# arneschneuing/DiffSBDD

Hardware: NVIDIA H100
Metric: ligand_atoms_per_sec_500step_ddpm (higher is better)
Workload: dtype f32

## Files before the change

### diffsbdd_b200/csrc/dsb_tc.cu

```cuda
#include "dsb_tc.cuh"

namespace dsb {
using namespace tc;

__global__ void pack_b_image_kernel(float* __restrict__ hi, float* __restrict__ lo, const float* __restrict__ src, int lds,
                                    int scol, int n_rows, int n_dst_off, int K, int chunks, int TN) {
  const int64_t idx = (int64_t)blockIdx.x * blockDim.x + threadIdx.x;
  if (idx >= (int64_t)n_rows * K) return;
  const int n = (int)(idx / K), k = (int)(idx - (int64_t)n * K);
  const int nd = n_dst_off + n, nt = nd / TN, nl = nd % TN;
  const int kc = k / TKC, c = (k % TKC) >> 2, j = k & 3;
  const size_t off = ((size_t)nt * chunks + kc) * (size_t)(TN * TKC) + sw128_offset(nl, c) / 4 + j;
  const float w = src[(size_t)n * lds + scol + k];
  const float h = tf32_hi(w);
  hi[off] = h;
  lo[off] = w - h;
}

void launch_pack_b_image(float* hi, float* lo, const float* src, int lds, int scol, int n_rows, int n_dst_off, int K, int tn) {
  const int64_t tot = (int64_t)n_rows * K;
  pack_b_image_kernel<<<(unsigned)((tot + 255) / 256), 256>>>(hi, lo, src, lds, scol, n_rows, n_dst_off, K, K / TKC, tn);
}

__global__ void pack_b_image_f16_kernel(__half* __restrict__ hi, __half* __restrict__ lo, const float* __restrict__ src, int lds,
                                        int scol, int n_rows, int n_dst_off, int K, int chunks, float scale, int TN) {
  const int64_t idx = (int64_t)blockIdx.x * blockDim.x + threadIdx.x;
  if (idx >= (int64_t)n_rows * K) return;
  const int n = (int)(idx / K), k = (int)(idx - (int64_t)n * K);
  const int nd = n_dst_off + n, nt = nd / TN, nl = nd % TN;
  const int kc = k / TKC16, c16 = (k % TKC16) >> 3, j = k & 7;
  const size_t off = ((size_t)nt * chunks + kc) * (size_t)(TN * 64) + sw128_offset(nl, c16) / 2 + j;
  const float w = src[(size_t)n * lds + scol + k] * scale;
  const __half h = __float2half_rn(w);
  hi[off] = h;
  lo[off] = __float2half_rn(w - __half2float(h));
}

void launch_pack_b_image_f16(float* hi, float* lo, const float* src, int lds, int scol, int n_rows, int n_dst_off, int K, float scale, int tn) {
  const int64_t tot = (int64_t)n_rows * K;
  pack_b_image_f16_kernel<<<(unsigned)((tot + 255) / 256), 256>>>(reinterpret_cast<__half*>(hi), reinterpret_cast<__half*>(lo), src,
                                                                  lds, scol, n_rows, n_dst_off, K, K / TKC16, scale, tn);
}

__global__ void absmax_kernel(const float* __restrict__ src, int lds, int scol, int n_rows, int K, unsigned* __restrict__ out) {
  const int64_t idx = (int64_t)blockIdx.x * blockDim.x + threadIdx.x;
  float v = 0.f;
  if (idx < (int64_t)n_rows * K) { const int n = (int)(idx / K), k = (int)(idx - (int64_t)n * K); v = fabsf(src[(size_t)n * lds + scol + k]); }
#pragma unroll
  for (int o = 16; o > 0; o >>= 1) v = fmaxf(v, __shfl_xor_sync(0xffffffffu, v, o));
  if ((threadIdx.x & 31) == 0) atomicMax(out, __float_as_uint(v));
}
void launch_absmax(const float* src, int lds, int scol, int n_rows, int K, unsigned* out) {
  const int64_t tot = (int64_t)n_rows * K;
  absmax_kernel<<<(unsigned)((tot + 255) / 256), 256>>>(src, lds, scol, n_rows, K, out);
}

constexpr size_t kControlBytes = 128;
static_assert(sizeof(Control) <= kControlBytes, "Control block grew");
__device__ __forceinline__ char* align1024(uint8_t* raw) {
  return reinterpret_cast<char*>(raw) + ((1024u - (smem_u32(raw) & 1023u)) & 1023u);
}
template <int H> constexpr size_t tc_smem_base() { return 1024 + (size_t)NSTAGE * Geo<H>::STAGE_BYTES + kControlBytes; }

struct TcGemmArgs {
  const float* A1; int lda1; int K1;
  const float* A2; int lda2; int K2; float div2; const int32_t* deg2;
  const float* Bhi; const float* Blo;
  const float* bias; const float* R; int ldr;
  float* C; int ldc; int M; int Nn; int act;
  float* Z; int ldz;
  int dead_mt; int dead_nt;
  float inv_scale;
};

struct TileMap {
  int ntn, ntm, dead_mt, dead_nt, nA, n_live;
  __device__ TileMap(int M, int Nn, int dmt, int dnt, int TN) {
    ntn = Nn / TN; ntm = (M + TM - 1) / TM;
    dead_nt = dnt; dead_mt = dnt > 0 ? (dmt < ntm ? dmt : ntm) : ntm;
    nA = dead_mt * ntn;
    n_live = nA + (ntm - dead_mt) * (ntn - dead_nt);
  }
  __device__ void get(int t, int& mt, int& nt) const {
    if (t < nA) { mt = t / ntn; nt = t - mt * ntn; }
    else { const int u = t - nA, w = ntn - dead_nt; mt = dead_mt + u / w; nt = dead_nt + (u - (u / w) * w); }
  }
};

template <TcFormat FMT, int H>
__global__ void __launch_bounds__(TC_THREADS, 1) tc_node_gemm_kernel(TcGemmArgs g) {
  using G = Geo<H>;
  constexpr bool F16 = FMT != TcFormat::TF32x3;
  constexpr int TN = H, HPC = F16 ? 2 : 1;
  extern __shared__ uint8_t smem_raw[];
  char* const stages = align1024(smem_raw);
  Control* ctl = reinterpret_cast<Control*>(stages + NSTAGE * G::STAGE_BYTES);
  const int wg = threadIdx.x >> 7, warp = (threadIdx.x >> 5) & 3, lane = threadIdx.x & 31;
  const TileMap tm(g.M, g.Nn, g.dead_mt, g.dead_nt, TN);
  const int n_tiles = tm.n_live;
  const int n_my = ((int)blockIdx.x < n_tiles) ? (n_tiles - (int)blockIdx.x + (int)gridDim.x - 1) / (int)gridDim.x : 0;
  if (n_my == 0) return;
  const int K = g.K1 + g.K2, chunks = K / (F16 ? TKC16 : TKC);
  const uint32_t total = (uint32_t)(n_my * chunks);
  pdl_trigger();
  if (threadIdx.x == 0) control_init(ctl);
  __syncthreads();
  pdl_wait();
  const WeightStream<FMT, H> wst{ctl, stages};
  auto issue_w = [&](uint32_t q) {
    const int it = (int)(q / chunks), kc = (int)(q - (uint32_t)it * chunks);
    int mt, nt;
    tm.get(blockIdx.x + it * gridDim.x, mt, nt);
    const size_t off = ((size_t)nt * chunks + kc) * G::B_CHUNK_FLOATS;
    wst.issue(q, g.Bhi + off, g.Blo + off);
  };
  if (threadIdx.x >= MMA_THREADS) {
    regs_dec<WEIGHT_WG_REGS>();
    if (threadIdx.x == MMA_THREADS)
      for (uint32_t q = 0; q < total; ++q) issue_w(q);
    return;
  }
  regs_inc<MMA_WG_REGS>();

  const int sr = lane >> 3, pc = lane & 7;
  const int r0 = wg * WG_ROWS + 16 * warp + 4 * sr;
  const int re = wg * WG_ROWS + 16 * warp + (lane >> 2);
  const bool divides = g.div2 != 1.0f || g.deg2 != nullptr;
  float acc[G::ACC];
  MmaTracker trk;
  uint32_t q = 0;
  for (int it = 0; it < n_my; ++it) {
    int mt, nt;
    tm.get(blockIdx.x + it * gridDim.x, mt, nt);
    const int m0 = mt * TM, n0 = nt * TN;
    for (int kc = 0; kc < chunks; ++kc, ++q) {
      const int s = q & 1;
      char* st = stages + (size_t)s * G::STAGE_BYTES;
#pragma unroll
      for (int h = 0; h < HPC; ++h) {
        const int hf = kc * HPC + h, k = hf * TKC + 4 * pc;
        const bool second = k >= g.K1;
        float4 v[4];
#pragma unroll
        for (int i = 0; i < 4; ++i) {
          const int m = m0 + r0 + i;
          v[i] = make_float4(0.f, 0.f, 0.f, 0.f);
          if (m < g.M) v[i] = second ? *reinterpret_cast<const float4*>(g.A2 + (size_t)m * g.lda2 + (k - g.K1))
                                     : *reinterpret_cast<const float4*>(g.A1 + (size_t)m * g.lda1 + k);
        }
#pragma unroll
        for (int i = 0; i < 4; ++i) {
          float4 x = v[i];
          if (second && divides) {
            const int m = m0 + r0 + i;
            const float dv = g.deg2 ? (float)max(m < g.M ? g.deg2[m] : 1, 1) : g.div2;
            x.x = __fdiv_rn(x.x, dv); x.y = __fdiv_rn(x.y, dv); x.z = __fdiv_rn(x.z, dv); x.w = __fdiv_rn(x.w, dv);
          }
          store_pair<FMT>(st + piece_offset<F16>(r0 + i, hf, pc), pk2(x.x, x.y), pk2(x.z, x.w));
        }
      }
      fence_proxy_async();
      wg_sync(wg);
      mbar_wait(&ctl->full_w[s], (q >> 1) & 1);
      wgmma_fence();
      mma_chunk<FMT, H>(acc, st, wg, kc == 0);
      wgmma_commit();
      trk.release_prev(ctl, (int)q, lane == 0);
    }
    trk.drain<H>(ctl, acc, lane == 0);
    const f32x2 ip = pk2(g.inv_scale, g.inv_scale);
#pragma unroll
    for (int j = 0; j < H / 8; ++j) {
      const int n = n0 + 8 * j + 2 * (lane & 3);
      const f32x2 b = g.bias ? *reinterpret_cast<const float2*>(g.bias + n) : pk2(0.f, 0.f);
#pragma unroll
      for (int hh = 0; hh < 2; ++hh) {
        f32x2 x = pk2(acc[4 * j + 2 * hh], acc[4 * j + 2 * hh + 1]);
        x = F16 ? fma2(x, ip, b) : add2(x, b);
        if (g.act == 1) x = silu2(x);
        upk2(x, acc[4 * j + 2 * hh], acc[4 * j + 2 * hh + 1]);
      }
    }
    if (g.R) {
#pragma unroll
      for (int j = 0; j < H / 8; ++j) {
        const int n = n0 + 8 * j + 2 * (lane & 3);
#pragma unroll
        for (int hh = 0; hh < 2; ++hh) {
          const int row = min(m0 + re + 8 * hh, g.M - 1);
          const f32x2 x = add2(*reinterpret_cast<const float2*>(g.R + (size_t)row * g.ldr + n),
                               pk2(acc[4 * j + 2 * hh], acc[4 * j + 2 * hh + 1]));
          upk2(x, acc[4 * j + 2 * hh], acc[4 * j + 2 * hh + 1]);
        }
      }
    }
    acc_fence(acc);
#pragma unroll
    for (int j = 0; j < H / 8; ++j) {
      const int n = n0 + 8 * j + 2 * (lane & 3);
#pragma unroll
      for (int hh = 0; hh < 2; ++hh) {
        const int row = m0 + re + 8 * hh;
        if (row < g.M) {
          *reinterpret_cast<float2*>(g.C + (size_t)row * g.ldc + n) = pk2(acc[4 * j + 2 * hh], acc[4 * j + 2 * hh + 1]);
          if (g.Z) *reinterpret_cast<float2*>(g.Z + (size_t)row * g.ldz + n) = make_float2(0.f, 0.f);
        }
      }
    }
  }
}

struct EdgeScalars {
  float d2[TM], d0[TM];
  int row[TM], col[TM], type[TM];
  float dir[3][TM];
};

template <int H>
struct EdgeExtra {
  float vec[2][3 * H];
  float wa[H];
  EdgeScalars sc[2];
};

struct TcEdgeArgs {
  const float* P; int ldp;
  const float4* x; const float4* cent; const int32_t* gid;
  const int32_t* vrow_ptr; const int32_t* vmap; int n_rows;
  const int32_t *erow, *ecol; const float* ed0; int NL;
  int nm;
  const float* W2hi[2]; const float* W2lo[2];
  const float* wr[2]; const float* wr0[2]; const float* tb[2]; const float* b2[2];
  const float* wa; const float* ba;
  float norm_constant, coords_range; int use_tanh;
  float* agg;
  float4* xagg;
  float inv_scale[2];
  float* part;
  int vcap;
};

template <bool COORD>
struct ScalarSteps {
  int e, r, c, gi;
  float d0;
  float4 xi, xj;
  __device__ __forceinline__ void step(int k, const TcEdgeArgs& a, EdgeScalars* sc, int pr, int v0, int V, int m) {
    if (k == 0) {
      const int vr = v0 + pr;
      e = a.vmap[min(vr, V - 1)];
      e = vr < V ? e : -1;
    } else if (k == 1) {
      const int ec = max(e, 0);
      r = a.erow[ec]; c = a.ecol[ec]; d0 = a.ed0[ec];
      r = e >= 0 ? r : 0; c = e >= 0 ? c : 0;
    } else if (k == 2) {
      xi = a.x[r]; xj = a.x[c];
      if (COORD) gi = a.gid[r];
    } else {
      const bool live = e >= 0;
      const float dx = xi.x - xj.x, dy = xi.y - xj.y, dz = xi.z - xj.z;
      const float d2 = dx * dx + dy * dy + dz * dz;
      const int ty = (r < a.NL) == (c < a.NL) ? (r < a.NL ? 1 : 2) : 0;
      sc->row[pr] = live ? r : -1; sc->col[pr] = c; sc->d2[pr] = live ? d2 : 0.f; sc->d0[pr] = live ? d0 : 0.f;
      sc->type[pr] = live ? ty : 0;
      if (COORD) {
        float dir[3];
        if (m == 0) {
          const float den = sqrtf(d2 + 1e-8f) + a.norm_constant;
          dir[0] = dx / den; dir[1] = dy / den; dir[2] = dz / den;
        } else {
          const float4 mu = a.cent[gi];
          const float ax = xi.x - mu.x, ay = xi.y - mu.y, az = xi.z - mu.z;
          const float bx = xj.x - mu.x, by = xj.y - mu.y, bz = xj.z - mu.z;
          const float cx = ay * bz - az * by, cy = az * bx - ax * bz, cz = ax * by - ay * bx;
          const float cn = sqrtf(cx * cx + cy * cy + cz * cz) + a.norm_constant;
          dir[0] = cx / cn; dir[1] = cy / cn; dir[2] = cz / cn;
        }
#pragma unroll
        for (int k = 0; k < 3; ++k) sc->dir[k][pr] = live ? dir[k] : 0.f;
      }
    }
  }
};

template <bool COORD, TcFormat FMT, int H, bool TB, bool DET = false>
__global__ void __launch_bounds__(TC_THREADS, 1) tc_edge_kernel(TcEdgeArgs a) {
  using G = Geo<H>;
  constexpr bool F16 = FMT != TcFormat::TF32x3;
  constexpr int HPC = F16 ? 2 : 1;
  constexpr int chunks = H / (TKC * HPC);
  extern __shared__ uint8_t smem_raw[];
  char* const stages = align1024(smem_raw);
  Control* ctl = reinterpret_cast<Control*>(stages + NSTAGE * G::STAGE_BYTES);
  EdgeExtra<H>* ex = reinterpret_cast<EdgeExtra<H>*>(reinterpret_cast<char*>(ctl) + kControlBytes);
  const int wg = threadIdx.x >> 7, wt = threadIdx.x & 127, warp = (threadIdx.x >> 5) & 3, lane = threadIdx.x & 31;
  const int nm = a.nm;

  pdl_trigger();
  for (int i = threadIdx.x; i < H; i += TC_THREADS) {
    for (int m = 0; m < nm; ++m) {
      float* v = ex->vec[m];
      v[i] = a.wr[m][i]; v[H + i] = a.wr0[m][i]; v[2 * H + i] = a.b2[m][i];
    }
    ex->wa[i] = a.wa ? a.wa[i] : 0.f;
  }
  if (threadIdx.x == 0) control_init(ctl);
  __syncthreads();
  pdl_wait();
  const int E = DET ? min(a.vrow_ptr[a.n_rows], a.vcap) : a.vrow_ptr[a.n_rows];
  const int n_units = ((E + TM - 1) / TM) * nm;
  const int n_my = ((int)blockIdx.x < n_units) ? (n_units - (int)blockIdx.x + (int)gridDim.x - 1) / (int)gridDim.x : 0;
  if (n_my == 0) return;
  auto unit_tile = [&](int j, int& m) { const int v = blockIdx.x + j * gridDim.x, t = v / nm; m = v - t * nm; return t; };
  const uint32_t total = (uint32_t)(n_my * chunks);
  const WeightStream<FMT, H> wst{ctl, stages};
  auto issue_w = [&](uint32_t q) {
    const int j = (int)(q / chunks), kc = (int)(q - (uint32_t)j * chunks);
    int m;
    unit_tile(j, m);
    wst.issue(q, a.W2hi[m] + (size_t)kc * G::B_CHUNK_FLOATS, a.W2lo[m] + (size_t)kc * G::B_CHUNK_FLOATS);
  };
  if (threadIdx.x >= MMA_THREADS) {
    regs_dec<WEIGHT_WG_REGS>();
    if (threadIdx.x == MMA_THREADS)
      for (uint32_t q = 0; q < total; ++q) issue_w(q);
    return;
  }
  regs_inc<MMA_WG_REGS>();

  const bool has_att = (!COORD) && a.wa != nullptr;
  const float ba = has_att ? a.ba[0] : 0.f;
  const int sr = lane >> 3, pc = lane & 7;
  const int r0 = wg * WG_ROWS + 16 * warp + 4 * sr;
  const int re = wg * WG_ROWS + 16 * warp + (lane >> 2);
  const float* const Pt = a.P + 4 * pc;
  const int soff = nm * H;
  auto build = [&](const EdgeScalars* sc, int m, int kc, int s) {
    char* st = stages + (size_t)s * G::STAGE_BYTES;
    const int moff = m * H;
    const float* pr = Pt + (size_t)max(sc->row[r0], 0) * a.ldp + moff;
    const int4 cl = *reinterpret_cast<const int4*>(sc->col + r0);
    const float4 d2v = *reinterpret_cast<const float4*>(sc->d2 + r0), d0v = *reinterpret_cast<const float4*>(sc->d0 + r0);
    const int4 tyv = *reinterpret_cast<const int4*>(sc->type + r0);
    const float* const ps[4] = {Pt + (size_t)cl.x * a.ldp + (soff + moff), Pt + (size_t)cl.y * a.ldp + (soff + moff),
                                Pt + (size_t)cl.z * a.ldp + (soff + moff), Pt + (size_t)cl.w * a.ldp + (soff + moff)};
    const float pd2[4] = {d2v.x, d2v.y, d2v.z, d2v.w}, pd0[4] = {d0v.x, d0v.y, d0v.z, d0v.w};
    const int pty[4] = {TB ? tyv.x * H : 0, TB ? tyv.y * H : 0, TB ? tyv.z * H : 0, TB ? tyv.w * H : 0};
    const float* wr = ex->vec[m] + 4 * pc;
    const float* wr0 = wr + H;
    const float* tbm = TB ? a.tb[m] + 4 * pc : nullptr;
#pragma unroll
    for (int h = 0; h < HPC; ++h) {
      const int hf = kc * HPC + h;
      const float4 ga = *reinterpret_cast<const float4*>(pr + hf * TKC);
      float4 gb[4];
#pragma unroll
      for (int i = 0; i < 4; ++i) gb[i] = *reinterpret_cast<const float4*>(ps[i] + hf * TKC);
      const float4 r4 = *reinterpret_cast<const float4*>(wr + hf * TKC);
      const float4 r04 = *reinterpret_cast<const float4*>(wr0 + hf * TKC);
      const f32x2 a01 = pk2(ga.x, ga.y), a23 = pk2(ga.z, ga.w);
#pragma unroll
      for (int i = 0; i < 4; ++i) {
        const f32x2 d2p = pk2(pd2[i], pd2[i]), d0p = pk2(pd0[i], pd0[i]);
        f32x2 u01 = fma2(d0p, pk2(r04.x, r04.y), fma2(d2p, pk2(r4.x, r4.y), add2(a01, pk2(gb[i].x, gb[i].y))));
        f32x2 u23 = fma2(d0p, pk2(r04.z, r04.w), fma2(d2p, pk2(r4.z, r4.w), add2(a23, pk2(gb[i].z, gb[i].w))));
        if (TB) {
          const float4 t4 = *reinterpret_cast<const float4*>(tbm + pty[i] + hf * TKC);
          u01 = add2(u01, pk2(t4.x, t4.y)); u23 = add2(u23, pk2(t4.z, t4.w));
        }
        silu_pair<(DSB_SILU_PAIR & 1) != 0, (DSB_SILU_QUAD & 1) != 0>(u01, u23);
        store_pair<FMT>(st + piece_offset<F16>(r0 + i, hf, pc), u01, u23);
      }
    }
  };
  float acc[G::ACC];
  MmaTracker trk;
  uint32_t q = 0;
  auto issue = [&](int kc) {
    const int s = q & 1;
    fence_proxy_async();
    wg_sync(wg);
    mbar_wait(&ctl->full_w[s], (q >> 1) & 1);
    wgmma_fence();
    mma_chunk<FMT, H>(acc, stages + (size_t)s * G::STAGE_BYTES, wg, kc == 0);
    wgmma_commit();
    trk.release_prev(ctl, (int)q, lane == 0);
    ++q;
  };
  static_assert(chunks >= 2, "the scalar steps of the next unit need at least one chunk before the last");
  constexpr int kSteps = 4;
  const int psc = wg * WG_ROWS + (wt & (WG_ROWS - 1));
  ScalarSteps<COORD> stp;
  int m;
  int e0 = unit_tile(0, m) * TM;
  for (int k = 0; k < kSteps; ++k) stp.step(k, a, &ex->sc[0], psc, e0, E, m);
  wg_sync(wg);
  build(&ex->sc[0], m, 0, 0);
  for (int j = 0; j < n_my; ++j) {
    const EdgeScalars* sc = &ex->sc[j & 1];
    EdgeScalars* sc_next = &ex->sc[(j + 1) & 1];
    int m_next;
    const int e0_next = unit_tile(j + 1, m_next) * TM;
#pragma unroll ((F16 && !(FMT == TcFormat::F16x1 && !COORD && TB && H == 256)) ? chunks : 1)
    for (int kc = 0; kc < chunks - 1; ++kc) {
      issue(kc);
      for (int k = kc * kSteps / (chunks - 1); k < (kc + 1) * kSteps / (chunks - 1); ++k)
        stp.step(k, a, sc_next, psc, e0_next, E, m_next);
      build(sc, m, kc + 1, q & 1);
    }
    issue(chunks - 1);
    build(sc_next, m_next, 0, q & 1);
    trk.drain<H>(ctl, acc, lane == 0);

    const float* b2 = ex->vec[m] + 2 * H;
    const f32x2 ip = pk2(a.inv_scale[m], a.inv_scale[m]);
    float s_lo = 0.f, s_hi = 0.f;
    if constexpr (DET) {
      static_assert((H / 8) % 2 == 0, "DET epilogue pairs column groups");
#pragma unroll
      for (int jj = 0; jj < H / 8; jj += 2) {
        const int c = 8 * jj + 2 * (lane & 3);
        const f32x2 b0 = *reinterpret_cast<const float2*>(b2 + c), b1 = *reinterpret_cast<const float2*>(b2 + c + 8);
        const float2 w0 = *reinterpret_cast<const float2*>(ex->wa + c), w1 = *reinterpret_cast<const float2*>(ex->wa + c + 8);
        f32x2 lo0 = pk2(acc[4 * jj], acc[4 * jj + 1]), lo1 = pk2(acc[4 * jj + 4], acc[4 * jj + 5]);
        f32x2 hi0 = pk2(acc[4 * jj + 2], acc[4 * jj + 3]), hi1 = pk2(acc[4 * jj + 6], acc[4 * jj + 7]);
        lo0 = F16 ? fma2(lo0, ip, b0) : add2(lo0, b0); lo1 = F16 ? fma2(lo1, ip, b1) : add2(lo1, b1);
        hi0 = F16 ? fma2(hi0, ip, b0) : add2(hi0, b0); hi1 = F16 ? fma2(hi1, ip, b1) : add2(hi1, b1);
        silu_pair<(DSB_SILU_PAIR & 2) != 0, (DSB_SILU_QUAD & 2) != 0>(lo0, lo1);
        silu_pair<(DSB_SILU_PAIR & 2) != 0, (DSB_SILU_QUAD & 2) != 0>(hi0, hi1);
        upk2(lo0, acc[4 * jj], acc[4 * jj + 1]); upk2(lo1, acc[4 * jj + 4], acc[4 * jj + 5]);
        upk2(hi0, acc[4 * jj + 2], acc[4 * jj + 3]); upk2(hi1, acc[4 * jj + 6], acc[4 * jj + 7]);
        s_lo = fmaf(lo0.y, w0.y, fmaf(lo0.x, w0.x, s_lo));
        s_lo = fmaf(lo1.y, w1.y, fmaf(lo1.x, w1.x, s_lo));
        s_hi = fmaf(hi0.y, w0.y, fmaf(hi0.x, w0.x, s_hi));
        s_hi = fmaf(hi1.y, w1.y, fmaf(hi1.x, w1.x, s_hi));
      }
    } else {
#pragma unroll
    for (int jj = 0; jj < H / 8; ++jj) {
      const int c = 8 * jj + 2 * (lane & 3);
      const f32x2 bb = *reinterpret_cast<const float2*>(b2 + c);
      const float2 ww = *reinterpret_cast<const float2*>(ex->wa + c);
      f32x2 lo = pk2(acc[4 * jj], acc[4 * jj + 1]), hi = pk2(acc[4 * jj + 2], acc[4 * jj + 3]);
      lo = F16 ? fma2(lo, ip, bb) : add2(lo, bb);
      hi = F16 ? fma2(hi, ip, bb) : add2(hi, bb);
      silu_pair<(DSB_SILU_PAIR & 2) != 0, (DSB_SILU_QUAD & 2) != 0>(lo, hi);
      upk2(lo, acc[4 * jj], acc[4 * jj + 1]); upk2(hi, acc[4 * jj + 2], acc[4 * jj + 3]);
      s_lo = fmaf(lo.y, ww.y, fmaf(lo.x, ww.x, s_lo));
      s_hi = fmaf(hi.y, ww.y, fmaf(hi.x, ww.x, s_hi));
    }
    }
    s_lo += __shfl_xor_sync(0xffffffffu, s_lo, 1); s_lo += __shfl_xor_sync(0xffffffffu, s_lo, 2);
    s_hi += __shfl_xor_sync(0xffffffffu, s_hi, 1); s_hi += __shfl_xor_sync(0xffffffffu, s_hi, 2);
    const int row_lo = sc->row[re], row_hi = sc->row[re + 8];
    const int crow_lo = sc->row[re & ~3], crow_hi = sc->row[(re + 8) & ~3];
    const bool chunk_lane = (lane & 12) == 0;
    if constexpr (!COORD) {
      float g_lo = has_att ? sigmoid_f(s_lo + ba) : 1.0f, g_hi = has_att ? sigmoid_f(s_hi + ba) : 1.0f;
      g_lo = row_lo >= 0 ? g_lo : 0.f;
      g_hi = row_hi >= 0 ? g_hi : 0.f;
      const bool hi_half = (lane & 4) != 0, odd_group = (lane & 8) != 0;
      const int crow = hi_half ? crow_hi : crow_lo;
      const int chunk_row = hi_half ? (re + 8) & ~3 : re & ~3;
      float* const dst = (DET ? a.part + (size_t)((e0 + chunk_row) / kRowChunk) * H : a.agg + (size_t)max(crow, 0) * H)
                         + 2 * (lane & 3) + (odd_group ? 8 : 0);
#pragma unroll
      for (int jj = 0; jj < H / 8; jj += 2) {
        const float lo[4] = {g_lo * acc[4 * jj], g_lo * acc[4 * jj + 1], g_lo * acc[4 * jj + 4], g_lo * acc[4 * jj + 5]};
        const float hi[4] = {g_hi * acc[4 * jj + 2], g_hi * acc[4 * jj + 3], g_hi * acc[4 * jj + 6], g_hi * acc[4 * jj + 7]};
        float t[4];
#pragma unroll
        for (int k = 0; k < 4; ++k) t[k] = (hi_half ? hi[k] : lo[k]) + __shfl_xor_sync(0xffffffffu, hi_half ? lo[k] : hi[k], 4);
        float u[2];
#pragma unroll
        for (int k = 0; k < 2; ++k) u[k] = (odd_group ? t[2 + k] : t[k]) + __shfl_xor_sync(0xffffffffu, odd_group ? t[k] : t[2 + k], 8);
        if constexpr (DET)
          asm volatile("st.global.v2.f32 [%0], {%1, %2};" ::"l"(dst + 8 * jj), "f"(u[0]), "f"(u[1]) : "memory");
        else
          asm volatile("red.global.add.v2.f32 [%0], {%1, %2};" ::"l"(dst + 8 * jj), "f"(u[0]), "f"(u[1]) : "memory");
      }
    } else {
#pragma unroll
      for (int hh = 0; hh < 2; ++hh) {
        const int r = re + 8 * hh;
        const float sv = hh ? s_hi : s_lo;
        const bool live = (hh ? row_hi : row_lo) >= 0;
        float tr[3];
#pragma unroll
        for (int k = 0; k < 3; ++k) {
          const float d = sc->dir[k][r];
          float t;
          if (m == 0) t = a.use_tanh ? (d * tanhf(sv)) * a.coords_range : d * sv;
          else t = d * (a.use_tanh ? tanhf(sv) * a.coords_range : sv);
          t = live ? t : 0.f;
          t += __shfl_xor_sync(0xffffffffu, t, 4);
          t += __shfl_xor_sync(0xffffffffu, t, 8);
          tr[k] = t;
        }
        const int crow = hh ? crow_hi : crow_lo;
        if constexpr (DET) {
          if (chunk_lane && (lane & 3) == 0)
            reinterpret_cast<float4*>(a.part)[(size_t)((e0 + (r & ~3)) / kRowChunk) * nm + m] = make_float4(tr[0], tr[1], tr[2], 0.f);
        } else if (chunk_lane && (lane & 3) == 0 && crow >= 0) {
#pragma unroll
          for (int k = 0; k < 3; ++k) atomicAdd(reinterpret_cast<float*>(a.xagg) + (size_t)crow * 4 + k, tr[k]);
        }
      }
    }
    m = m_next; e0 = e0_next;
  }
}

template <int H> static size_t gemm_smem_bytes() { return tc_smem_base<H>(); }
template <int H> static size_t edge_smem_bytes() {
  static_assert(tc_smem_base<H>() + sizeof(EdgeExtra<H>) <= 232448, "edge kernel exceeds the 227 KB of shared memory per CTA");
  return tc_smem_base<H>() + sizeof(EdgeExtra<H>);
}

bool tc_width_supported(int H) { return H == 128 || H == 192 || H == 256; }

template <typename Fn>
static int dispatch_width(int H, Fn&& fn) {
  switch (H) {
    case 128: return fn.template operator()<128>();
    case 192: return fn.template operator()<192>();
    case 256: return fn.template operator()<256>();
    default: set_error("tensor-core kernels exist for hidden_nf 128, 192, 256 (got %d)", H); return DSB_ERR_UNSUPPORTED_CONFIG;
  }
}

template <typename Fn>
static int dispatch_tc(TcFormat f, int H, Fn&& fn) {
  return dispatch_width(H, [&]<int W>() -> int {
    switch (f) {
      case TcFormat::TF32x3: return fn.template operator()<TcFormat::TF32x3, W>();
      case TcFormat::F16x3: return fn.template operator()<TcFormat::F16x3, W>();
      default: return fn.template operator()<TcFormat::F16x1, W>();
    }
  });
}

int configure_tc_kernels(int H) {
  for (const TcFormat f : {TcFormat::TF32x3, TcFormat::F16x3, TcFormat::F16x1}) {
    const int e = dispatch_tc(f, H, [&]<TcFormat F, int W>() -> int {
      const int gs = (int)gemm_smem_bytes<W>(), es = (int)edge_smem_bytes<W>();
      DSB_CUDA_OK(cudaFuncSetAttribute(tc_node_gemm_kernel<F, W>, cudaFuncAttributeMaxDynamicSharedMemorySize, gs));
      DSB_CUDA_OK(cudaFuncSetAttribute(tc_edge_kernel<false, F, W, false>, cudaFuncAttributeMaxDynamicSharedMemorySize, es));
      DSB_CUDA_OK(cudaFuncSetAttribute(tc_edge_kernel<false, F, W, true>, cudaFuncAttributeMaxDynamicSharedMemorySize, es));
      DSB_CUDA_OK(cudaFuncSetAttribute(tc_edge_kernel<true, F, W, false>, cudaFuncAttributeMaxDynamicSharedMemorySize, es));
      DSB_CUDA_OK(cudaFuncSetAttribute(tc_edge_kernel<true, F, W, true>, cudaFuncAttributeMaxDynamicSharedMemorySize, es));
      DSB_CUDA_OK(cudaFuncSetAttribute(tc_edge_kernel<false, F, W, false, true>, cudaFuncAttributeMaxDynamicSharedMemorySize, es));
      DSB_CUDA_OK(cudaFuncSetAttribute(tc_edge_kernel<false, F, W, true, true>, cudaFuncAttributeMaxDynamicSharedMemorySize, es));
      DSB_CUDA_OK(cudaFuncSetAttribute(tc_edge_kernel<true, F, W, false, true>, cudaFuncAttributeMaxDynamicSharedMemorySize, es));
      DSB_CUDA_OK(cudaFuncSetAttribute(tc_edge_kernel<true, F, W, true, true>, cudaFuncAttributeMaxDynamicSharedMemorySize, es));
      return 0;
    });
    if (e) return e;
  }
  return 0;
}

int launch_tc_node_gemm(const dsb_dynamics* d, const GemmArgs& g, const TcImage& w, int n_tile_off, TcFormat fmt, int32_t* status,
                        cudaStream_t s) {
  (void)status;
  if (g.M == 0) return 0;
  const bool f16 = fmt != TcFormat::TF32x3;
  const int K = g.K1 + g.K2, TN = d->cfg.hidden_nf;
  if ((g.Nn % TN) || (K % TKC16) || (g.K1 % TKC16) || (g.lda1 % 4) || (g.ldc % 4)) {
    set_error("tc_node_gemm: unsupported shape K1=%d K2=%d Nn=%d", g.K1, g.K2, g.Nn);
    return DSB_ERR_INVALID_ARGUMENT;
  }
  TcGemmArgs a;
  a.A1 = g.A1; a.lda1 = g.lda1; a.K1 = g.K1; a.A2 = g.A2; a.lda2 = g.lda2; a.K2 = g.K2; a.div2 = g.div2; a.deg2 = g.deg2;
  const size_t img_off = (size_t)n_tile_off * (K / (f16 ? TKC16 : TKC)) * (size_t)(TN * TKC);
  a.Bhi = (f16 ? w.h_hi : w.t_hi) + img_off; a.Blo = (f16 ? w.h_lo : w.t_lo) + img_off;
  a.Z = g.Z; a.ldz = g.ldz;
  a.dead_nt = g.dead_cols / TN; a.dead_mt = a.dead_nt > 0 ? (g.dead_rows_from + TM - 1) / TM : 0;
  a.bias = g.bias; a.R = g.R; a.ldr = g.ldr; a.C = g.C; a.ldc = g.ldc; a.M = g.M; a.Nn = g.Nn; a.act = g.act;
  a.inv_scale = f16 ? w.h_inv : 1.0f;
  const int ntn_ = g.Nn / TN, ntm_ = (g.M + TM - 1) / TM;
  const int dmt_ = a.dead_nt > 0 ? (a.dead_mt < ntm_ ? a.dead_mt : ntm_) : ntm_;
  const int n_tiles = dmt_ * ntn_ + (ntm_ - dmt_) * (ntn_ - a.dead_nt);
  const int grid = n_tiles < d->num_sms ? n_tiles : d->num_sms;
  return dispatch_tc(fmt, TN, [&]<TcFormat F, int W>() -> int {
    DSB_CUDA_OK(launch_k(tc_node_gemm_kernel<F, W>, grid, TC_THREADS, gemm_smem_bytes<W>(), s, a));
    return 0;
  });
}

int launch_tc_edge_gcl(const dsb_dynamics* d, const Dims& dm, const Workspace& ws, const GclW& w, const float4* x, PView pv, TcFormat fmt,
                       int32_t* status, cudaStream_t s) {
  (void)status;
  const bool f16 = fmt != TcFormat::TF32x3;
  TcEdgeArgs a = {};
  a.P = pv.P; a.ldp = pv.ldp; a.x = x; a.cent = ws.cent; a.gid = ws.gid; a.vrow_ptr = ws.vrow_ptr; a.vmap = ws.vmap; a.n_rows = dm.N;
  a.erow = ws.erow; a.ecol = ws.ecol; a.ed0 = ws.ed0; a.NL = dm.NL; a.nm = 1;
  a.W2hi[0] = f16 ? w.iW2.h_hi : w.iW2.t_hi; a.W2lo[0] = f16 ? w.iW2.h_lo : w.iW2.t_lo;
  a.inv_scale[0] = f16 ? w.iW2.h_inv : 1.0f; a.inv_scale[1] = 1.0f;
  a.wr[0] = w.wr; a.wr0[0] = w.wr0; a.tb[0] = w.tb; a.b2[0] = w.b2;
  a.wa = w.wa; a.ba = w.ba; a.agg = ws.agg; a.part = ws.part; a.vcap = ws.vcap;
  const bool det = d->deterministic != 0;
  return dispatch_tc(fmt, d->cfg.hidden_nf, [&]<TcFormat F, int W>() -> int {
    auto kern = w.tb ? tc_edge_kernel<false, F, W, true> : tc_edge_kernel<false, F, W, false>;
    if (det) kern = w.tb ? tc_edge_kernel<false, F, W, true, true> : tc_edge_kernel<false, F, W, false, true>;
    DSB_CUDA_OK(launch_k(kern, d->num_sms, TC_THREADS, edge_smem_bytes<W>(), s, a));
    return 0;
  });
}

int launch_tc_edge_coord(const dsb_dynamics* d, const Dims& dm, const Workspace& ws, const EquivW& w, const float4* x, PView pv, TcFormat fmt,
                         int32_t* status, cudaStream_t s) {
  (void)status;
  const bool f16 = fmt != TcFormat::TF32x3;
  const dsb_config& c = d->cfg;
  TcEdgeArgs a = {};
  a.nm = c.reflection_equivariant ? 1 : 2;
  a.P = pv.P; a.ldp = pv.ldp; a.x = x; a.cent = ws.cent; a.gid = ws.gid; a.vrow_ptr = ws.vrow_ptr; a.vmap = ws.vmap; a.n_rows = dm.n_coord_rows;
  a.erow = ws.erow; a.ecol = ws.ecol; a.ed0 = ws.ed0; a.NL = dm.NL;
  a.inv_scale[0] = a.inv_scale[1] = 1.0f;
  for (int m = 0; m < a.nm; ++m) {
    a.W2hi[m] = f16 ? w.iW2[m].h_hi : w.iW2[m].t_hi; a.W2lo[m] = f16 ? w.iW2[m].h_lo : w.iW2[m].t_lo;
    a.inv_scale[m] = f16 ? w.iW2[m].h_inv : 1.0f;
    a.wr[m] = w.wr[m]; a.wr0[m] = w.wr0[m]; a.tb[m] = w.tb[m]; a.b2[m] = w.b2[m];
  }
  a.wa = w.w3; a.ba = nullptr;
  a.norm_constant = c.norm_constant; a.coords_range = c.coords_range; a.use_tanh = c.tanh; a.xagg = ws.xagg; a.part = ws.part; a.vcap = ws.vcap;
  const bool det = d->deterministic != 0;
  return dispatch_tc(fmt, c.hidden_nf, [&]<TcFormat F, int W>() -> int {
    auto kern = w.tb[0] ? tc_edge_kernel<true, F, W, true> : tc_edge_kernel<true, F, W, false>;
    if (det) kern = w.tb[0] ? tc_edge_kernel<true, F, W, true, true> : tc_edge_kernel<true, F, W, false, true>;
    DSB_CUDA_OK(launch_k(kern, d->num_sms, TC_THREADS, edge_smem_bytes<W>(), s, a));
    return 0;
  });
}

}
```

### profiles/node_gemm_breakdown.py

```python
from __future__ import annotations

import argparse
import json
import os
import statistics
import subprocess
import sys

import torch

ROOT = os.path.dirname(os.path.dirname(os.path.abspath(__file__)))
sys.path.insert(0, ROOT)

import bench
from diffsbdd_b200 import synthetic as syn
from diffsbdd_b200.dynamics import EGNNDynamics

TM = 128
PEAK_TFLOPS = {'3xfp16': 989.0, '3xtf32': 495.0}
HBM_TBS = 3.35


def gpu_info():
    try:
        out = subprocess.run(['nvidia-smi', '--id=0', '--query-gpu=name,power.limit,clocks.sm,clocks.max.sm',
                              '--format=csv,noheader'], capture_output=True, text=True, timeout=30).stdout.strip()
        return out
    except Exception:
        return None


def launch_plan(cfg, n, n_lig):
    H = cfg.hidden_nf
    nm = 1 if cfg.reflection_equivariant else 2
    conditional = not cfg.update_pocket_coords
    plan = []
    for layer in range(cfg.n_layers):
        for sub in range(cfg.inv_sublayers):
            if not (sub == 0 and layer > 0):
                plan.append(('g1', H, 2 * H, False, False, 0, 0))
            plan.append(('g2', 2 * H, H, False, False, 0, 0))
            plan.append(('g3', H, H, True, True, 0, 0))
        plan.append(('g4', H, nm * 2 * H + 2 * H, False, False, n_lig if conditional else 0, nm * H if conditional else 0))
    return plan


def shape_counts(H, M, K, Nn, has_r, has_z, dead_from, dead_cols, f16, n_sms):
    ntn, ntm = Nn // H, (M + TM - 1) // TM
    dnt = dead_cols // H
    dmt = min((dead_from + TM - 1) // TM, ntm) if dnt > 0 else ntm
    tiles = dmt * ntn + (ntm - dmt) * (ntn - dnt)
    chunks = K // (64 if f16 else 32)
    dead_rows = max(M - dmt * TM, 0) if dnt > 0 else 0
    c_elems = M * Nn - dead_rows * dnt * H
    hbm = 4 * (M * K + (M * Nn if has_r else 0) + c_elems + (M * H if has_z else 0))
    return {'tiles': tiles, 'ctas': min(tiles, n_sms), 'chunks_per_tile': chunks,
            'exec_gflop': 6.0 * tiles * TM * H * K / 1e9, 'hbm_lb_mb': hbm / 1e6,
            'l2_weight_mb': tiles * chunks * 2 * H * 128 / 1e6}


def profile_workload(name, calls, warmup, math_mode, flush):
    a = argparse.Namespace(workload=name)
    cfg, _, _, _ = bench.workload(a)
    _, B, NL, NP, _, _, _, _ = bench.WORKLOADS[name]
    sd = syn.synthetic_state_dict(cfg, 0)
    dyn = EGNNDynamics.from_config(cfg, device='cuda')
    dyn.load_state_dict(sd)
    dyn.eval()
    dyn.math_mode = math_mode
    inp = [x.cuda() for x in syn.synthetic_denoiser_inputs(cfg, [NL] * B, [NP] * B, seed=1)]
    H, M = cfg.hidden_nf, B * (NL + NP)
    plan = launch_plan(cfg, M, B * NL)
    with torch.no_grad():
        for _ in range(warmup):
            bench.l2_flush(flush)
            dyn(*inp)
        torch.cuda.synchronize()
        with torch.profiler.profile(activities=[torch.profiler.ProfilerActivity.CUDA]) as prof:
            for _ in range(calls):
                bench.l2_flush(flush)
                dyn(*inp)
            torch.cuda.synchronize()
    raw = sorted(((e.start_ns(), e.start_ns() + e.duration_ns(), e.name()) for e in prof.profiler.kineto_results.events()
                  if e.device_type() == torch.autograd.DeviceType.CUDA), key=lambda t: t[0])
    kern, last_end = [], 0
    for s, e, n in raw:
        kern.append((s, max(e - max(s, last_end), 0), n, e - s))
        last_end = max(last_end, e)
    gemms = [k for k in kern if 'tc_node_gemm_kernel' in k[2]]
    if len(gemms) != calls * len(plan):
        raise SystemExit(f'{name}: {len(gemms)} node-GEMM kernels for {calls} calls, expected {len(plan)} per call')
    per_label, span = {}, {}
    for i, (_, dur, _, sp) in enumerate(gemms):
        per_label.setdefault(plan[i % len(plan)][0], []).append(dur / 1e3)
        span.setdefault(plan[i % len(plan)][0], []).append(sp / 1e3)
    classes = {'node_gemm': 'tc_node_gemm_kernel', 'edge_gcl': 'tc_edge_kernel<false', 'edge_coord': 'tc_edge_kernel<true'}
    by_class = {c: round(sum(d for _, d, n, _ in kern if key in n) / 1e6 / calls, 4) for c, key in classes.items()}
    by_class['all_dsb_kernels'] = round(sum(d for _, d, n, _ in kern if 'dsb::' in n) / 1e6 / calls, 4)
    f16 = math_mode == '3xfp16'
    rows = []
    for lab in ('g1', 'g2', 'g3', 'g4'):
        if lab not in per_label:
            continue
        p = next(x for x in plan if x[0] == lab)
        sc = shape_counts(H, M, p[1], p[2], p[3], p[4], p[5], p[6], f16, torch.cuda.get_device_properties(0).multi_processor_count)
        us = statistics.median(per_label[lab])
        rows.append({'label': lab, 'launches_per_call': len(per_label[lab]) // calls, 'M': M, 'K': p[1], 'Nn': p[2],
                     'us_median': round(us, 2), 'us_min': round(min(per_label[lab]), 2), 'us_max': round(max(per_label[lab]), 2),
                     'span_us_median': round(statistics.median(span[lab]), 2),
                     **sc, 'exec_tflops': round(sc['exec_gflop'] / us * 1e3, 1),
                     'tensor_bound_us': round(sc['exec_gflop'] / PEAK_TFLOPS[math_mode] / 1e-3, 2),
                     'hbm_bound_us': round(sc['hbm_lb_mb'] / HBM_TBS, 2),
                     'l2_weight_gbs': round(sc['l2_weight_mb'] / us * 1e3, 1)})
    node_ms = sum(r['us_median'] * r['launches_per_call'] for r in rows) / 1e3
    return {'workload': name, 'hidden_nf': H, 'M': M, 'math_mode': math_mode, 'calls': calls,
            'node_gemm_ms_per_call_from_medians': round(node_ms, 4), 'ms_per_call_by_class': by_class, 'per_label': rows}


def print_table(res):
    print(f"\n{res['workload']} (H = {res['hidden_nf']}, M = {res['M']}, {res['math_mode']}); per call: {res['ms_per_call_by_class']}")
    print('| launch | per call | us/launch (min-max) | span us | tiles | CTAs | exec TFLOP/s | tensor bound us | HBM LB MB | HBM bound us '
          '| L2 weight MB | L2 weight GB/s |')
    print('|---|---|---|---|---|---|---|---|---|---|---|---|')
    for r in res['per_label']:
        print(f"| {r['label']} | {r['launches_per_call']} | {r['us_median']} ({r['us_min']}-{r['us_max']}) | {r['span_us_median']} | {r['tiles']} | {r['ctas']} "
              f"| {r['exec_tflops']} | {r['tensor_bound_us']} | {r['hbm_lb_mb']:.1f} | {r['hbm_bound_us']} | {r['l2_weight_mb']:.1f} "
              f"| {r['l2_weight_gbs']} |")


def main():
    ap = argparse.ArgumentParser()
    ap.add_argument('--workloads', default='fullatom,moad,moad_ca')
    ap.add_argument('--calls', type=int, default=20)
    ap.add_argument('--warmup', type=int, default=5)
    ap.add_argument('--math-mode', default='3xfp16', choices=sorted(PEAK_TFLOPS))
    ap.add_argument('--out', default=None)
    args = ap.parse_args()
    if not torch.cuda.is_available():
        raise SystemExit('node_gemm_breakdown.py needs a CUDA device')
    flush = torch.zeros(64 * 1024 * 1024, dtype=torch.float32, device='cuda')
    out = {'gpu': gpu_info(), 'torch_device': torch.cuda.get_device_name(0), 'results': []}
    print('gpu (name, power limit, SM clock, max SM clock):', out['gpu'])
    for w in args.workloads.split(','):
        res = profile_workload(w, args.calls, args.warmup, args.math_mode, flush)
        out['results'].append(res)
        print_table(res)
    print('\n(tensor / HBM bounds: data-sheet peaks of a 700 W H100 SXM, not measured; DRAM traffic is not measured)')
    if args.out:
        with open(args.out, 'w') as f:
            json.dump(out, f, indent=1)


if __name__ == '__main__':
    main()
```

Baseline: 962.5.

## Prefetch A chunks one step ahead and issue weight loads before PDL wait

For hidden sizes above 128, the node GEMM kernel now software-pipelines the activation loads: the next chunk's A tile, or the next tile's first chunk, is loaded into registers while the current one is stored and multiplied. Out-of-range row reads are clamped so the loads need no branch. The weight producer thread issues the first NSTAGE weight chunks before the programmatic-dependent-launch wait, overlapping that fetch with the tail of the previous kernel. The MMA warpgroups now wait on PDL only after raising their register allocation. This raises register pressure and assumes the packed weights are not written by the preceding kernel. The profiling script also reports tiles per CTA.

New measurement: 977.0, median of 6. +1.5%, better.

```diff
diff --git a/diffsbdd_b200/csrc/dsb_tc.cu b/diffsbdd_b200/csrc/dsb_tc.cu
--- a/diffsbdd_b200/csrc/dsb_tc.cu
+++ b/diffsbdd_b200/csrc/dsb_tc.cu
@@ -105,7 +105,6 @@
   pdl_trigger();
   if (threadIdx.x == 0) control_init(ctl);
   __syncthreads();
-  pdl_wait();
   const WeightStream<FMT, H> wst{ctl, stages};
   auto issue_w = [&](uint32_t q) {
     const int it = (int)(q / chunks), kc = (int)(q - (uint32_t)it * chunks);
@@ -114,51 +113,87 @@
     const size_t off = ((size_t)nt * chunks + kc) * G::B_CHUNK_FLOATS;
     wst.issue(q, g.Bhi + off, g.Blo + off);
   };
+  constexpr bool AHEAD = H > 128;
   if (threadIdx.x >= MMA_THREADS) {
     regs_dec<WEIGHT_WG_REGS>();
-    if (threadIdx.x == MMA_THREADS)
-      for (uint32_t q = 0; q < total; ++q) issue_w(q);
+    if (threadIdx.x == MMA_THREADS) {
+      uint32_t q = 0;
+      for (; q < total && q < (AHEAD ? (uint32_t)NSTAGE : 0u); ++q) issue_w(q);
+      pdl_wait();
+      for (; q < total; ++q) issue_w(q);
+    }
     return;
   }
   regs_inc<MMA_WG_REGS>();
+  pdl_wait();
 
   const int sr = lane >> 3, pc = lane & 7;
   const int r0 = wg * WG_ROWS + 16 * warp + 4 * sr;
   const int re = wg * WG_ROWS + 16 * warp + (lane >> 2);
   const bool divides = g.div2 != 1.0f || g.deg2 != nullptr;
+  auto load_a = [&](float4 (&v)[HPC][4], int m0, int kc) {
+#pragma unroll
+    for (int h = 0; h < HPC; ++h) {
+      const int k = (kc * HPC + h) * TKC + 4 * pc;
+      const bool second = k >= g.K1;
+#pragma unroll
+      for (int i = 0; i < 4; ++i) {
+        const int m = m0 + r0 + i;
+        if constexpr (AHEAD) {
+          const float* const src = second ? g.A2 + (k - g.K1) : g.A1 + k;
+          v[h][i] = *reinterpret_cast<const float4*>(src + (size_t)min(m, g.M - 1) * (second ? g.lda2 : g.lda1));
+        } else {
+          v[h][i] = make_float4(0.f, 0.f, 0.f, 0.f);
+          if (m < g.M) v[h][i] = second ? *reinterpret_cast<const float4*>(g.A2 + (size_t)m * g.lda2 + (k - g.K1))
+                                        : *reinterpret_cast<const float4*>(g.A1 + (size_t)m * g.lda1 + k);
+        }
+      }
+    }
+  };
+  auto store_a = [&](const float4 (&v)[HPC][4], int m0, int kc, char* st) {
+#pragma unroll
+    for (int h = 0; h < HPC; ++h) {
+      const int hf = kc * HPC + h, k = hf * TKC + 4 * pc;
+      const bool second = k >= g.K1;
+#pragma unroll
+      for (int i = 0; i < 4; ++i) {
+        const int m = m0 + r0 + i;
+        float4 x = (!AHEAD || m < g.M) ? v[h][i] : make_float4(0.f, 0.f, 0.f, 0.f);
+        if (second && divides) {
+          const float dv = g.deg2 ? (float)max(m < g.M ? g.deg2[m] : 1, 1) : g.div2;
+          x.x = __fdiv_rn(x.x, dv); x.y = __fdiv_rn(x.y, dv); x.z = __fdiv_rn(x.z, dv); x.w = __fdiv_rn(x.w, dv);
+        }
+        store_pair<FMT>(st + piece_offset<F16>(r0 + i, hf, pc), pk2(x.x, x.y), pk2(x.z, x.w));
+      }
+    }
+  };
   float acc[G::ACC];
   MmaTracker trk;
   uint32_t q = 0;
+  float4 va[HPC][4];
+  int mt, nt;
+  tm.get(blockIdx.x, mt, nt);
+  if constexpr (AHEAD) load_a(va, mt * TM, 0);
   for (int it = 0; it < n_my; ++it) {
-    int mt, nt;
     tm.get(blockIdx.x + it * gridDim.x, mt, nt);
     const int m0 = mt * TM, n0 = nt * TN;
+    int mt_next = mt, nt_next;
+    if (AHEAD && it + 1 < n_my) tm.get(blockIdx.x + (it + 1) * gridDim.x, mt_next, nt_next);
     for (int kc = 0; kc < chunks; ++kc, ++q) {
       const int s = q & 1;
       char* st = stages + (size_t)s * G::STAGE_BYTES;
-#pragma unroll
-      for (int h = 0; h < HPC; ++h) {
-        const int hf = kc * HPC + h, k = hf * TKC + 4 * pc;
-        const bool second = k >= g.K1;
-        float4 v[4];
-#pragma unroll
-        for (int i = 0; i < 4; ++i) {
-          const int m = m0 + r0 + i;
-          v[i] = make_float4(0.f, 0.f, 0.f, 0.f);
-          if (m < g.M) v[i] = second ? *reinterpret_cast<const float4*>(g.A2 + (size_t)m * g.lda2 + (k - g.K1))
-                                     : *reinterpret_cast<const float4*>(g.A1 + (size_t)m * g.lda1 + k);
-        }
-#pragma unroll
-        for (int i = 0; i < 4; ++i) {
-          float4 x = v[i];
-          if (second && divides) {
-            const int m = m0 + r0 + i;
-            const float dv = g.deg2 ? (float)max(m < g.M ? g.deg2[m] : 1, 1) : g.div2;
-            x.x = __fdiv_rn(x.x, dv); x.y = __fdiv_rn(x.y, dv); x.z = __fdiv_rn(x.z, dv); x.w = __fdiv_rn(x.w, dv);
-          }
-          store_pair<FMT>(st + piece_offset<F16>(r0 + i, hf, pc), pk2(x.x, x.y), pk2(x.z, x.w));
-        }
-      }
+      float4 v[HPC][4];
+      if constexpr (AHEAD) {
+#pragma unroll
+        for (int h = 0; h < HPC; ++h)
+#pragma unroll
+          for (int i = 0; i < 4; ++i) v[h][i] = va[h][i];
+        if (kc + 1 < chunks) load_a(va, m0, kc + 1);
+        else load_a(va, mt_next * TM, 0);
+      } else {
+        load_a(v, m0, kc);
+      }
+      store_a(v, m0, kc, st);
       fence_proxy_async();
       wg_sync(wg);
       mbar_wait(&ctl->full_w[s], (q >> 1) & 1);
diff --git a/profiles/node_gemm_breakdown.py b/profiles/node_gemm_breakdown.py
--- a/profiles/node_gemm_breakdown.py
+++ b/profiles/node_gemm_breakdown.py
@@ -54,7 +54,9 @@
     dead_rows = max(M - dmt * TM, 0) if dnt > 0 else 0
     c_elems = M * Nn - dead_rows * dnt * H
     hbm = 4 * (M * K + (M * Nn if has_r else 0) + c_elems + (M * H if has_z else 0))
-    return {'tiles': tiles, 'ctas': min(tiles, n_sms), 'chunks_per_tile': chunks,
+    ctas = min(tiles, n_sms)
+    return {'tiles': tiles, 'ctas': ctas, 'tiles_per_cta_max': -(-tiles // ctas), 'tiles_per_cta_mean': round(tiles / ctas, 2),
+            'chunks_per_tile': chunks,
             'exec_gflop': 6.0 * tiles * TM * H * K / 1e9, 'hbm_lb_mb': hbm / 1e6,
             'l2_weight_mb': tiles * chunks * 2 * H * 128 / 1e6}
 
@@ -119,11 +121,12 @@
 
 def print_table(res):
     print(f"\n{res['workload']} (H = {res['hidden_nf']}, M = {res['M']}, {res['math_mode']}); per call: {res['ms_per_call_by_class']}")
-    print('| launch | per call | us/launch (min-max) | span us | tiles | CTAs | exec TFLOP/s | tensor bound us | HBM LB MB | HBM bound us '
-          '| L2 weight MB | L2 weight GB/s |')
-    print('|---|---|---|---|---|---|---|---|---|---|---|---|')
+    print('| launch | per call | us/launch (min-max) | span us | tiles | CTAs | tiles/CTA (most, mean) | exec TFLOP/s | tensor bound us '
+          '| HBM LB MB | HBM bound us | L2 weight MB | L2 weight GB/s |')
+    print('|---|---|---|---|---|---|---|---|---|---|---|---|---|')
     for r in res['per_label']:
         print(f"| {r['label']} | {r['launches_per_call']} | {r['us_median']} ({r['us_min']}-{r['us_max']}) | {r['span_us_median']} | {r['tiles']} | {r['ctas']} "
+              f"| {r['tiles_per_cta_max']}, {r['tiles_per_cta_mean']} "
               f"| {r['exec_tflops']} | {r['tensor_bound_us']} | {r['hbm_lb_mb']:.1f} | {r['hbm_bound_us']} | {r['l2_weight_mb']:.1f} "
               f"| {r['l2_weight_gbs']} |")
 
```
